# hanzz2007/libxsmm-1

Hardware: AMD Instinct MI355X
Metric: batched SMM fp32 32x32x32 GFLOP/s (whole job) (higher is better)
Workload: dtype f32; 1 GPU; configs[1]: batched dense SMM fp32 M=N=K=32 alpha=1 beta=1, batch=1048576 per GPU, strided addressing, MFMA on; batch_per_gpu=1048576, parallelism=batch-shard x1

## Files before the change

include/libxsmm_amd.h:

```cpp
#ifndef LIBXSMM_AMD_H
#define LIBXSMM_AMD_H

#if !defined(LIBXSMM_H)
# include "libxsmm.h"
#endif

LIBXSMM_API int libxsmm_amd_device_count(void);
LIBXSMM_API void libxsmm_amd_set_stream(void* hip_stream);
LIBXSMM_API void* libxsmm_amd_get_stream(void);
LIBXSMM_API void libxsmm_amd_defer_begin(void);
LIBXSMM_API void libxsmm_amd_defer_end(void);
LIBXSMM_API int libxsmm_amd_defer_active(void);
LIBXSMM_API void libxsmm_amd_flush(void);
LIBXSMM_API int libxsmm_amd_merge_segments(int n, const unsigned long long hulls[], int segment_of[]);
LIBXSMM_API int libxsmm_amd_merge_last_plan(int* ncalls, int* nsegments, int* ndevice_hulls, unsigned long long hulls[], int segment_of[], int capacity);
LIBXSMM_API int libxsmm_amd_smm_plan_describe(const libxsmm_gemm_descriptor* descriptor, int mode, int sync, long long batch,
  long long stride_a, long long stride_b, long long stride_c, unsigned int address_bits, int relaxed, long long uniform_run, int mfma, int lowp,
  char* buffer, size_t buffer_size, int compile_tiles);
LIBXSMM_API int libxsmm_amd_synchronize(void);
LIBXSMM_API void* libxsmm_amd_device_malloc(size_t size);
LIBXSMM_API void libxsmm_amd_device_free(void* ptr);
LIBXSMM_API int libxsmm_amd_memcpy_h2d(void* dst_device, const void* src_host, size_t size);
LIBXSMM_API int libxsmm_amd_memcpy_d2h(void* dst_host, const void* src_device, size_t size);
LIBXSMM_API int libxsmm_amd_is_device_pointer(const void* ptr);

LIBXSMM_API int libxsmm_amd_set_mfma(int mode);
LIBXSMM_API int libxsmm_amd_get_mfma(void);
LIBXSMM_API const char* libxsmm_amd_last_kernel(void);
LIBXSMM_API unsigned long long libxsmm_amd_launch_count(void);
LIBXSMM_API unsigned long long libxsmm_amd_jit_launch_count(void);

LIBXSMM_API int libxsmm_amd_stream_probe(const void* a, const void* b, void* c, long long bytes);

LIBXSMM_API int libxsmm_amd_gemm_batch_strided(const libxsmm_gemm_descriptor* descriptor,
  const void* a, const void* b, void* c, long long stride_a, long long stride_b, long long stride_c,
  long long batchsize);

LIBXSMM_API int libxsmm_amd_gemm_batch_groups(libxsmm_gemm_precision iprec, libxsmm_gemm_precision oprec, int ngroups,
  const char transa[], const char transb[], const libxsmm_blasint m[], const libxsmm_blasint n[], const libxsmm_blasint k[],
  const libxsmm_blasint lda[], const libxsmm_blasint ldb[], const libxsmm_blasint ldc[], const void* alpha, const void* beta,
  const void* const a[], const void* const b[], void* const c[], libxsmm_blasint index_base, libxsmm_blasint index_stride,
  const libxsmm_blasint* const stride_a[], const libxsmm_blasint* const stride_b[], const libxsmm_blasint* const stride_c[],
  const libxsmm_blasint group_size[], int relaxed);

typedef struct libxsmm_amd_spmdm_batch libxsmm_amd_spmdm_batch;
LIBXSMM_API libxsmm_amd_spmdm_batch* libxsmm_amd_spmdm_batch_create(int M, int N, int K, long long batch);
LIBXSMM_API void libxsmm_amd_spmdm_batch_destroy(libxsmm_amd_spmdm_batch* sb);
LIBXSMM_API int libxsmm_amd_spmdm_batch_create_slices(libxsmm_amd_spmdm_batch* sb, char transa, const float* a);
LIBXSMM_API int libxsmm_amd_spmdm_batch_compute(libxsmm_amd_spmdm_batch* sb, char transb, const float* b,
  char transc, const float* beta, float* c);
LIBXSMM_API int libxsmm_amd_spmdm_batch_get_slice(const libxsmm_amd_spmdm_batch* sb, long long item,
  uint16_t* rowidx, uint16_t* colidx, float* values, int capacity);

LIBXSMM_API int libxsmm_amd_spmdm_createSparseSlice_all(const libxsmm_spmdm_handle* handle, char transa, const float* a,
  libxsmm_CSR_sparseslice* libxsmm_output_csr_a);
LIBXSMM_API int libxsmm_amd_spmdm_compute_all(const libxsmm_spmdm_handle* handle, char transa, char transb, const float* alpha,
  libxsmm_CSR_sparseslice* a_sparse, const float* b, char transc, const float* beta, float* c);
LIBXSMM_API int libxsmm_amd_spmdm_createSparseSlice_bfloat16_all(const libxsmm_spmdm_handle* handle, char transa, const libxsmm_bfloat16* a,
  libxsmm_CSR_sparseslice* libxsmm_output_csr_a);
LIBXSMM_API int libxsmm_amd_spmdm_compute_bfloat16_all(const libxsmm_spmdm_handle* handle, char transa, char transb, const libxsmm_bfloat16* alpha,
  libxsmm_CSR_sparseslice* a_sparse, const libxsmm_bfloat16* b, char transc, const libxsmm_bfloat16* beta, float* c);

LIBXSMM_API int libxsmm_amd_dfsspmdm_execute_batch(const libxsmm_dfsspmdm* handle, const double* B, double* C, long long batch);
LIBXSMM_API int libxsmm_amd_sfsspmdm_execute_batch(const libxsmm_sfsspmdm* handle, const float* B, float* C, long long batch);

LIBXSMM_API int libxsmm_amd_csr_kernel_source(int typesize, int M, int K, const unsigned int* row_ptr, const unsigned int* column_idx,
  const double* values, int beta0, int vec, char* buffer, size_t buffer_size, int compile);

LIBXSMM_API int libxsmm_amd_smm_kernel_source(const libxsmm_gemm_descriptor* descriptor, int variant, char* buffer, size_t buffer_size, int compile);

LIBXSMM_API int libxsmm_amd_smm_grouped_kernel_source(const libxsmm_gemm_descriptor* const descriptors[], int ndescriptors, char* buffer, size_t buffer_size, int compile);

LIBXSMM_API void libxsmm_amd_jit_wait(void);
LIBXSMM_API void libxsmm_amd_jit_drain(void);
LIBXSMM_API int libxsmm_amd_jit_prebuild(const libxsmm_gemm_descriptor* const descriptors[], int ndescriptors, int grouped);

typedef struct libxsmm_amd_spgemm libxsmm_amd_spgemm;
LIBXSMM_API libxsmm_amd_spgemm* libxsmm_amd_spgemm_create(const libxsmm_gemm_descriptor* descriptor, int is_csr,
  const unsigned int* row_idx, const unsigned int* column_idx, int fma);
LIBXSMM_API int libxsmm_amd_spgemm_execute_batch(const libxsmm_amd_spgemm* handle, const void* sparse_values, const void* dense, void* c,
  long long stride_dense, long long stride_c, long long batch);
LIBXSMM_API void libxsmm_amd_spgemm_destroy(const libxsmm_amd_spgemm* handle);
LIBXSMM_API int libxsmm_amd_spgemm_source(const libxsmm_gemm_descriptor* descriptor, int is_csr, const unsigned int* row_idx,
  const unsigned int* column_idx, int fma, char* buffer, size_t buffer_size, int compile);
LIBXSMM_API int libxsmm_amd_soa_source(const libxsmm_gemm_descriptor* descriptor, int form, const unsigned int* ptr, const unsigned int* idx,
  int fma, char* buffer, size_t buffer_size, int compile);

LIBXSMM_API int libxsmm_amd_sparse_reader(const char* path, int is_csr, unsigned int** o_ptr, unsigned int** o_idx, double** o_values,
  unsigned int* o_row_count, unsigned int* o_column_count, unsigned int* o_element_count);

LIBXSMM_API int libxsmm_amd_soa_width(libxsmm_gemm_precision precision);
LIBXSMM_API int libxsmm_amd_kernel_execute_batch(const void* kernel, const void* a, const void* b, void* c,
  long long stride_dense, long long stride_c, long long batch);

LIBXSMM_API int libxsmm_amd_packed_width(unsigned int typesize);
LIBXSMM_API int libxsmm_amd_packed_execute_batch(const void* kernel, const void* a, const void* b, void* c, long long npacks);
LIBXSMM_API int libxsmm_amd_packed_kernel_source(const void* descriptor, int kind, char* buffer, size_t buffer_size, int compile);

LIBXSMM_API int libxsmm_amd_matcopy_batch(void* out, const void* in, unsigned int typesize, libxsmm_blasint m, libxsmm_blasint n,
  libxsmm_blasint ldi, libxsmm_blasint ldo, long long stride_in, long long stride_out, long long batch);
LIBXSMM_API int libxsmm_amd_otrans_batch(void* out, const void* in, unsigned int typesize, libxsmm_blasint m, libxsmm_blasint n,
  libxsmm_blasint ldi, libxsmm_blasint ldo, long long stride_in, long long stride_out, long long batch);
LIBXSMM_API int libxsmm_amd_matcopy_batch_ptr(void* const out[], const void* const in[], unsigned int typesize, libxsmm_blasint m,
  libxsmm_blasint n, libxsmm_blasint ldi, libxsmm_blasint ldo, long long batch);
LIBXSMM_API int libxsmm_amd_otrans_batch_ptr(void* const out[], const void* const in[], unsigned int typesize, libxsmm_blasint m,
  libxsmm_blasint n, libxsmm_blasint ldi, libxsmm_blasint ldo, long long batch);

LIBXSMM_API int libxsmm_amd_gemm_task(const libxsmm_gemm_handle* handle, int tid, int nthreads, unsigned int rect[4]);
LIBXSMM_API int libxsmm_amd_gemm_tile(void);

LIBXSMM_API int libxsmm_amd_lowp_gemm(libxsmm_gemm_precision iprec, libxsmm_gemm_precision oprec, char transa, char transb,
  libxsmm_blasint m, libxsmm_blasint n, libxsmm_blasint k, const void* a, libxsmm_blasint lda, const void* b, libxsmm_blasint ldb,
  int beta, void* c, libxsmm_blasint ldc);
LIBXSMM_API int libxsmm_amd_lowp_gemm_thread(libxsmm_gemm_precision iprec, libxsmm_gemm_precision oprec, char transa, char transb,
  libxsmm_blasint m, libxsmm_blasint n, libxsmm_blasint k, const void* a, libxsmm_blasint lda, const void* b, libxsmm_blasint ldb,
  int beta, void* c, libxsmm_blasint ldc, int tid, int nthreads);
LIBXSMM_API int libxsmm_amd_set_lowp_fast(int on);
LIBXSMM_API int libxsmm_amd_get_lowp_fast(void);
LIBXSMM_API int libxsmm_amd_lowp_gemm_chunk(libxsmm_gemm_precision iprec);

LIBXSMM_API int libxsmm_amd_dnn_quantize_async(float* in_buffer, short* out_buffer, int length, unsigned char add_shift, unsigned char* scf, int round_mode);
LIBXSMM_API int libxsmm_amd_dnn_quantize_act_async(float* in_buffer, short* out_buffer, unsigned int N, unsigned int C, unsigned int H, unsigned int W,
  unsigned int cblk_f32, unsigned int cblk_i16, unsigned int lp_blk, unsigned char add_shift, unsigned char* scf, int round_mode);
LIBXSMM_API int libxsmm_amd_dnn_quantize_fil_async(float* in_buffer, short* out_buffer, unsigned int K, unsigned int C, unsigned int R, unsigned int S,
  unsigned int cblk_f32, unsigned int cblk_i16, unsigned int kblk_f32, unsigned int kblk_i16, unsigned int lp_blk, unsigned char add_shift,
  unsigned char* scf, int round_mode);
LIBXSMM_API void libxsmm_amd_dnn_quantize_set_seed(unsigned int seed);

LIBXSMM_API int libxsmm_amd_matdiff_async(libxsmm_matdiff_info* info, libxsmm_datatype datatype, libxsmm_blasint m, libxsmm_blasint n,
  const void* ref, const void* tst, const libxsmm_blasint* ldref, const libxsmm_blasint* ldtst);
LIBXSMM_API int libxsmm_amd_matdiff_batch(libxsmm_matdiff_info* info, libxsmm_matdiff_info* items, long long* item, libxsmm_datatype datatype,
  libxsmm_blasint m, libxsmm_blasint n, const void* ref, const void* tst, const libxsmm_blasint* ldref, const libxsmm_blasint* ldtst,
  long long stride_ref, long long stride_tst, long long batch);

#endif
```

libxsmm-1_amd/csrc/kernels/smm_special.hip:

```cpp
#include "smm_common.cuh"
#include <mutex>

namespace xsmm {
namespace {

typedef float f32x4 __attribute__((ext_vector_type(4)));
typedef float f32x16 __attribute__((ext_vector_type(16)));
typedef double f64x4 __attribute__((ext_vector_type(4)));

__device__ __forceinline__ bool aligned16(const void* p) { return 0 == (reinterpret_cast<uintptr_t>(p) & 15); }

template<bool GLB> struct Space { typedef float* ptr; typedef const float* cptr; typedef f32x4* vptr; typedef const f32x4* cvptr; };
template<> struct Space<true> {
  typedef __attribute__((address_space(1))) float* ptr; typedef const __attribute__((address_space(1))) float* cptr;
  typedef __attribute__((address_space(1))) f32x4* vptr; typedef const __attribute__((address_space(1))) f32x4* cvptr;
};
template<bool NT, bool GLB> __device__ __forceinline__ f32x4 ld4(const float* p, bool al)
{
  const typename Space<GLB>::cptr g = (typename Space<GLB>::cptr)p;
  if (al) return NT ? __builtin_nontemporal_load((typename Space<GLB>::cvptr)g) : *(typename Space<GLB>::cvptr)g;
  return f32x4{ g[0], g[1], g[2], g[3] };
}
template<bool NT, bool GLB> __device__ __forceinline__ void st4(float* p, bool al, f32x4 v)
{
  const typename Space<GLB>::ptr g = (typename Space<GLB>::ptr)p;
  if (al) { if (NT) __builtin_nontemporal_store(v, (typename Space<GLB>::vptr)g); else *(typename Space<GLB>::vptr)g = v; }
  else { g[0] = v[0]; g[1] = v[1]; g[2] = v[2]; g[3] = v[3]; }
}
template<bool NT, bool GLB> __device__ __forceinline__ float ld1(const float* p) { const typename Space<GLB>::cptr g = (typename Space<GLB>::cptr)p; return NT ? __builtin_nontemporal_load(g) : *g; }
template<bool NT, bool GLB> __device__ __forceinline__ void st1(float* p, float v) { const typename Space<GLB>::ptr g = (typename Space<GLB>::ptr)p; if (NT) __builtin_nontemporal_store(v, g); else *g = v; }

template<bool NT, bool GLB> __device__ __forceinline__ void load_mat32(const float* p, int lane, f32x4 (&r)[4])
{
  const bool al = aligned16(p);
#pragma unroll
  for (int j = 0; j < 4; ++j) r[j] = ld4<NT, GLB>(p + 4 * (64 * j + lane), al);
}

template<int KEYSHIFT> __device__ __forceinline__ void park_ab(float* As, float* Bs, int lane, const f32x4 (&ra)[4], const f32x4 (&rb)[4])
{
#pragma unroll
  for (int j = 0; j < 4; ++j) {
    const int c = 64 * j + lane;
    *reinterpret_cast<f32x4*>(As + 4 * c) = ra[j];
    const int n = c >> 3, q = c & 7;
    *reinterpret_cast<f32x4*>(Bs + 4 * (n * 8 + (q ^ ((n >> KEYSHIFT) & 7)))) = rb[j];
  }
}

template<bool BETA0, bool NT, bool GLB>
__global__ __launch_bounds__(256, 4)
void smm32_f32_fma_kernel(DevAddr ad, long long batch)
{
  __shared__ __align__(16) float lds[4][2048];
  const int wave = __builtin_amdgcn_readfirstlane(threadIdx.x >> 6), lane = threadIdx.x & 63;
  const int tx = lane & 7, ty = lane >> 3;
  float* const As = lds[wave];
  float* const Bs = lds[wave] + 1024;
  const long long w = (long long)blockIdx.x * 4 + wave, W = (long long)gridDim.x * 4;
  if (w >= batch) return;

  f32x4 ra[4], rb[4], rc[4];
  load_mat32<NT, GLB>(addr_a<float>(ad, w), lane, ra);
  load_mat32<NT, GLB>(addr_b<float>(ad, w), lane, rb);
  if (!BETA0) {
    const float* const pc = addr_c<float>(ad, w) + 4 * ty * 32 + 4 * tx;
    const bool al = aligned16(pc);
#pragma unroll
    for (int j = 0; j < 4; ++j) rc[j] = ld4<NT, GLB>(pc + j * 32, al);
  }
  for (long long item = w; item < batch; item += W) {
    float* const pc = addr_c<float>(ad, item) + 4 * ty * 32 + 4 * tx;
    park_ab<2>(As, Bs, lane, ra, rb);
    f32x4 acc[4];
#pragma unroll
    for (int j = 0; j < 4; ++j) acc[j] = BETA0 ? f32x4{ 0.f, 0.f, 0.f, 0.f } : rc[j];
    const long long next = item + W;
    if (next < batch) {
      load_mat32<NT, GLB>(addr_a<float>(ad, next), lane, ra);
      load_mat32<NT, GLB>(addr_b<float>(ad, next), lane, rb);
      if (!BETA0) {
        const float* const pn = addr_c<float>(ad, next) + 4 * ty * 32 + 4 * tx;
        const bool al = aligned16(pn);
#pragma unroll
        for (int j = 0; j < 4; ++j) rc[j] = ld4<NT, GLB>(pn + j * 32, al);
      }
    }
    wave_lds_sync();
#pragma unroll 2
    for (int q = 0; q < 8; ++q) {
      f32x4 av[4], bv[4];
#pragma unroll
      for (int kk = 0; kk < 4; ++kk) av[kk] = *reinterpret_cast<const f32x4*>(As + (4 * q + kk) * 32 + 4 * tx);
#pragma unroll
      for (int j = 0; j < 4; ++j) bv[j] = *reinterpret_cast<const f32x4*>(Bs + 4 * ((4 * ty + j) * 8 + (q ^ ty)));
#pragma unroll
      for (int kk = 0; kk < 4; ++kk) {
#pragma unroll
        for (int j = 0; j < 4; ++j) {
#pragma unroll
          for (int i = 0; i < 4; ++i) acc[j][i] = xfma(av[kk][i], bv[j][kk], acc[j][i]);
        }
      }
    }
    const bool al = aligned16(pc);
#pragma unroll
    for (int j = 0; j < 4; ++j) st4<NT, GLB>(pc + j * 32, al, acc[j]);
    wave_lds_sync();
  }
}

template<bool BETA0, bool NT, bool GLB, bool RUNS>
__global__ __launch_bounds__(256, 4)
void smm32_f32_mfma_kernel(DevAddr ad, long long batch, int runlen)
{
  __shared__ __align__(16) float lds[4][2048];
  const int wave = __builtin_amdgcn_readfirstlane(threadIdx.x >> 6), lane = threadIdx.x & 63;
  const int lo = lane & 31, hi = lane >> 5;
  float* const As = lds[wave];
  float* const Bs = lds[wave] + 1024;
  const long long w = (long long)blockIdx.x * 4 + wave, W = (long long)gridDim.x * 4;
  const long long nunits = RUNS ? batch / runlen : batch;
  if (w >= nunits) return;
  const int coff = 4 * hi * 32 + lo;

  f32x4 ra[4], rb[4];
  float rc[16];
  auto load_c = [&](const float* pc) {
#pragma unroll
    for (int r = 0; r < 16; ++r) rc[r] = ld1<NT, GLB>(pc + ((r & 3) + 8 * (r >> 2)) * 32);
  };
  long long unit = w;
  int r0 = 0;
  auto step = [&](long long u, int r, long long& u1, int& r1) { r1 = RUNS ? r + 1 : 0; u1 = u; if (!RUNS || r1 == runlen) { r1 = 0; u1 += W; } };
  float* pc_cur; float* pc_nxt = nullptr;
  {
    const long long first = RUNS ? unit * runlen : unit;
    load_mat32<NT, GLB>(addr_a<float>(ad, first), lane, ra);
    load_mat32<NT, GLB>(addr_b<float>(ad, first), lane, rb);
    pc_cur = addr_c<float>(ad, first);
    if (!BETA0) load_c(pc_cur + coff);
  }
  long long raw_a = 0, raw_b = 0, raw_c = 0;
  if (!RUNS && unit + W < nunits) {
    raw_a = raw_of(ad.a, ad.ia, ad.sa, ad, unit + W); raw_b = raw_of(ad.b, ad.ib, ad.sb, ad, unit + W); raw_c = raw_of(ad.c, ad.ic, ad.sc, ad, unit + W);
  }
  f32x16 acc;
  f32x16 pend; float* pend_pc = nullptr;
  auto store_pend = [&]() {
#pragma unroll
    for (int r = 0; r < 16; ++r) st1<NT, GLB>(pend_pc + ((r & 3) + 8 * (r >> 2)) * 32, pend[r]);
  };
  for (;;) {
    __builtin_amdgcn_s_waitcnt(0x0F70);
    if (nullptr != pend_pc) { store_pend(); pend_pc = nullptr; }
    park_ab<1>(As, Bs, lane, ra, rb);
    if (!RUNS || 0 == r0) {
#pragma unroll
      for (int r = 0; r < 16; ++r) acc[r] = BETA0 ? 0.f : rc[r];
    }
    int r1; long long unit1; step(unit, r0, unit1, r1);
    const bool more = unit1 < nunits;
    if (more) {
      if (RUNS) {
        const long long next = unit1 * runlen + r1;
        load_mat32<NT, GLB>(addr_a<float>(ad, next), lane, ra);
        load_mat32<NT, GLB>(addr_b<float>(ad, next), lane, rb);
        if (0 == r1) { pc_nxt = addr_c<float>(ad, next); if (!BETA0) load_c(pc_nxt + coff); } else pc_nxt = pc_cur;
      }
      else {
        load_mat32<NT, GLB>(cooked<const float>(ad.a, ad, raw_a), lane, ra);
        load_mat32<NT, GLB>(cooked<const float>(ad.b, ad, raw_b), lane, rb);
        pc_nxt = cooked<float>(ad.c, ad, raw_c);
        if (!BETA0) load_c(pc_nxt + coff);
        const long long next2 = unit1 + W;
        if (next2 < nunits) { raw_a = raw_of(ad.a, ad.ia, ad.sa, ad, next2); raw_b = raw_of(ad.b, ad.ib, ad.sb, ad, next2); raw_c = raw_of(ad.c, ad.ic, ad.sc, ad, next2); }
      }
    }
    wave_lds_sync();
    f32x4 bt[8];
#pragma unroll
    for (int t = 0; t < 8; ++t) bt[t] = *reinterpret_cast<const f32x4*>(Bs + 4 * (lo * 8 + (t ^ ((lo >> 1) & 7))));
#pragma unroll
    for (int s = 0; s < 16; ++s) {
      const float av = As[(2 * s + hi) * 32 + lo];
      const float bv = (0 != hi) ? bt[s >> 1][2 * (s & 1) + 1] : bt[s >> 1][2 * (s & 1)];
      acc = __builtin_amdgcn_mfma_f32_32x32x2f32(bv, av, acc, 0, 0, 0);
    }
    if (!RUNS || r0 + 1 == runlen) { pend = acc; pend_pc = pc_cur + coff; }
    wave_lds_sync();
    if (!more) break;
    unit = unit1; r0 = r1; pc_cur = pc_nxt;
  }
  if (nullptr != pend_pc) store_pend();
}

template<bool BETA0>
__global__ __launch_bounds__(256, 4)
void smm64_f32_mfma_kernel(DevAddr ad, long long batch)
{
  __shared__ __align__(16) float As[4096];
  __shared__ __align__(16) float Bs[4096];
  const int t = threadIdx.x, wave = __builtin_amdgcn_readfirstlane(t >> 6), lane = t & 63, lo = lane & 31, hi = lane >> 5;
  const int mq = wave & 1, nq = wave >> 1;
  const int m = 32 * mq + lo, n = 32 * nq + lo;
  const int coff = (32 * nq + 4 * hi) * 64 + m;
  long long item = blockIdx.x;
  if (item >= batch) return;

  f32x4 ra[4], rb[4];
  float rc[16];
  auto load_ab = [&](long long i) {
    const float* const pa = addr_a<float>(ad, i);
    const float* const pb = addr_b<float>(ad, i);
    const bool ala = aligned16(pa), alb = aligned16(pb);
#pragma unroll
    for (int j = 0; j < 4; ++j) {
      ra[j] = ld4<true, false>(pa + 4 * (256 * j + t), ala);
      rb[j] = ld4<true, false>(pb + 4 * (256 * j + t), alb);
    }
  };
  auto load_c = [&](const float* pc) {
#pragma unroll
    for (int r = 0; r < 16; ++r) rc[r] = ld1<true, false>(pc + ((r & 3) + 8 * (r >> 2)) * 64);
  };
  load_ab(item);
  if (!BETA0) load_c(addr_c<float>(ad, item) + coff);
  for (; item < batch; item += gridDim.x) {
    float* const pc = addr_c<float>(ad, item) + coff;
#pragma unroll
    for (int j = 0; j < 4; ++j) {
      const int c = 256 * j + t, row = c >> 4, q = c & 15;
      *reinterpret_cast<f32x4*>(As + row * 64 + ((4 * q) ^ ((row & 1) << 5))) = ra[j];
      *reinterpret_cast<f32x4*>(Bs + row * 64 + 4 * (q ^ (row & 15))) = rb[j];
    }
    f32x16 acc;
#pragma unroll
    for (int r = 0; r < 16; ++r) acc[r] = BETA0 ? 0.f : rc[r];
    const long long next = item + gridDim.x;
    if (next < batch) {
      load_ab(next);
      if (!BETA0) load_c(addr_c<float>(ad, next) + coff);
    }
    __syncthreads();
#pragma unroll
    for (int half = 0; half < 2; ++half) {
      f32x4 bt[8];
#pragma unroll
      for (int u = 0; u < 8; ++u) bt[u] = *reinterpret_cast<const f32x4*>(Bs + n * 64 + 4 * ((8 * half + u) ^ (n & 15)));
#pragma unroll
      for (int s = 0; s < 16; ++s) {
        const float av = As[(32 * half + 2 * s + hi) * 64 + (m ^ (hi << 5))];
        const float bv = (0 != hi) ? bt[s >> 1][2 * (s & 1) + 1] : bt[s >> 1][2 * (s & 1)];
        acc = __builtin_amdgcn_mfma_f32_32x32x2f32(bv, av, acc, 0, 0, 0);
      }
    }
#pragma unroll
    for (int r = 0; r < 16; ++r) st1<true, false>(pc + ((r & 3) + 8 * (r >> 2)) * 64, acc[r]);
    __syncthreads();
  }
}

#include "smm_mfma_wg.inc"

__global__ __launch_bounds__(256)
void stream_abc_kernel(const f32x4* __restrict__ a, const f32x4* __restrict__ b, f32x4* __restrict__ c, long long items)
{
  const int lane = threadIdx.x & 63;
  const long long w = (long long)blockIdx.x * (blockDim.x >> 6) + __builtin_amdgcn_readfirstlane(threadIdx.x >> 6), W = ((long long)gridDim.x * blockDim.x) >> 6;
  if (w >= items) return;
  f32x4 ra[4], rb[4], rc[4];
#pragma unroll
  for (int j = 0; j < 4; ++j) {
    const long long o = w * 256 + 64 * j + lane;
    ra[j] = __builtin_nontemporal_load(a + o); rb[j] = __builtin_nontemporal_load(b + o); rc[j] = __builtin_nontemporal_load(c + o);
  }
  for (long long it = w; it < items; it += W) {
    f32x4 r[4];
#pragma unroll
    for (int j = 0; j < 4; ++j) r[j] = ra[j] + rb[j] + rc[j];
    const long long nx = it + W;
    if (nx < items) {
#pragma unroll
      for (int j = 0; j < 4; ++j) {
        const long long o = nx * 256 + 64 * j + lane;
        ra[j] = __builtin_nontemporal_load(a + o); rb[j] = __builtin_nontemporal_load(b + o); rc[j] = __builtin_nontemporal_load(c + o);
      }
    }
#pragma unroll
    for (int j = 0; j < 4; ++j) __builtin_nontemporal_store(r[j], c + it * 256 + 64 * j + lane);
  }
}

int env_int(const char* name, int fallback)
{
  const char* const v = getenv(name);
  return (nullptr != v && 0 != *v) ? atoi(v) : fallback;
}

bool is_smm32_f32(const SmmBatch& s)
{
  return 4 == s.typesize && 32 == s.m && 32 == s.n && 32 == s.k && 32 == s.lda && 32 == s.ldb && 32 == s.ldc
      && 0 == (s.flags & LIBXSMM_GEMM_FLAG_TRANS_B) && SYNC_NONE == s.sync && 0 == s.general;
}

bool is_smm64(const SmmBatch& s, int typesize)
{
  return typesize == s.typesize && 64 == s.m && 64 == s.n && 64 == s.k && 64 == s.lda && 64 == s.ldb && 64 == s.ldc
      && 0 == (s.flags & LIBXSMM_GEMM_FLAG_TRANS_B) && SYNC_NONE == s.sync && 0 == s.general && 0 != s.use_mfma;
}

long long mfma_wg_units(const SmmBatch& s)
{
  if (SYNC_NONE == s.sync) return s.batch;
  if (SYNC_RUNS == s.sync && 0 < s.uniform_run && 0 == s.batch % s.uniform_run) return s.batch / s.uniform_run;
  return 0;
}
int mfma_wg_runlen(const SmmBatch& s) { return SYNC_NONE == s.sync ? 1 : s.uniform_run; }

template<bool NT, bool GLB>
int launch_smm32(const SmmBatch& s, hipStream_t st, unsigned blocks, const char** name)
{
  const bool beta0 = (0 != (s.flags & LIBXSMM_GEMM_FLAG_BETA_0));
  const DevAddr ad = make_addr(s);
  if (0 == s.use_mfma) {
    *name = "smm_f32_32x32x32_fma";
    if (beta0) hipLaunchKernelGGL((smm32_f32_fma_kernel<true, NT, GLB>), dim3(blocks), dim3(256), 0, st, ad, s.batch);
    else hipLaunchKernelGGL((smm32_f32_fma_kernel<false, NT, GLB>), dim3(blocks), dim3(256), 0, st, ad, s.batch);
  }
  else {
    *name = "smm_f32_32x32x32_mfma";
    if (beta0) hipLaunchKernelGGL((smm32_f32_mfma_kernel<true, NT, GLB, false>), dim3(blocks), dim3(256), 0, st, ad, s.batch, 1);
    else hipLaunchKernelGGL((smm32_f32_mfma_kernel<false, NT, GLB, false>), dim3(blocks), dim3(256), 0, st, ad, s.batch, 1);
  }
  return (int)hipGetLastError();
}

}

int launch_smm_special(const SmmBatch& s, void* stream, const char** name)
{
  hipStream_t st = (hipStream_t)stream;
  if (is_smm32_f32(s)) {
    const int bpc = env_int("XSMM_SMM32_BPC", (ADDR_STRIDED == s.mode || 0 == s.use_mfma) ? 3 : 4), nt = env_int("XSMM_SMM32_NT", 1);
    const int variant = env_int("XSMM_SMM32_VARIANT", 0 != s.use_mfma ? 0 : 1);
    long long blocks = (s.batch + 3) / 4;
    const int grid_env = env_int("XSMM_SMM32_GRID", 0);
    const long long resident = (0 < grid_env) ? grid_env : 256LL * (bpc > 0 ? bpc : 3);
    if (blocks > resident) blocks = resident;
    if (1 == variant) return (0 != nt) ? launch_smm32<true, true>(s, st, (unsigned)blocks, name) : launch_smm32<false, true>(s, st, (unsigned)blocks, name);
    return (0 != nt) ? launch_smm32<true, false>(s, st, (unsigned)blocks, name) : launch_smm32<false, false>(s, st, (unsigned)blocks, name);
  }
  if (4 == s.typesize && 32 == s.m && 32 == s.n && 32 == s.k && 32 == s.lda && 32 == s.ldb && 32 == s.ldc && 0 == (s.flags & LIBXSMM_GEMM_FLAG_TRANS_B)
    && SYNC_RUNS == s.sync && 0 < s.uniform_run && 0 == s.batch % s.uniform_run && 0 == s.general && 0 != s.use_mfma && 0 != env_int("XSMM_SMM32_RUNS", 1))
  {
    const long long units = s.batch / s.uniform_run;
    const int bpc = env_int("XSMM_SMM32_RUNS_BPC", 4);
    long long blocks = (units + 3) / 4;
    const long long resident = 256LL * (bpc > 0 ? bpc : 4);
    if (blocks > resident) blocks = resident;
    if (blocks < 1) return -1;
    const DevAddr ad = make_addr(s);
    *name = "smm_f32_32x32x32_mfma_runs";
    if (0 != (s.flags & LIBXSMM_GEMM_FLAG_BETA_0)) hipLaunchKernelGGL((smm32_f32_mfma_kernel<true, false, true, true>), dim3((unsigned)blocks), dim3(256), 0, st, ad, s.batch, s.uniform_run);
    else hipLaunchKernelGGL((smm32_f32_mfma_kernel<false, false, true, true>), dim3((unsigned)blocks), dim3(256), 0, st, ad, s.batch, s.uniform_run);
    return (int)hipGetLastError();
  }
  if (is_smm64(s, 4) && 0 != env_int("XSMM_SMM64_MFMA", 1) && 0 != env_int("XSMM_SMM64_TIGHT", 1)) {
    const int bpc = env_int("XSMM_SMM64_BPC", 4);
    long long blocks = s.batch;
    const long long resident = 256LL * (bpc > 0 ? bpc : 3);
    if (blocks > resident) blocks = resident;
    if (blocks < 1) return -1;
    const DevAddr ad = make_addr(s);
    *name = "smm_f32_64x64x64_mfma";
    if (0 != (s.flags & LIBXSMM_GEMM_FLAG_BETA_0)) hipLaunchKernelGGL((smm64_f32_mfma_kernel<true>), dim3((unsigned)blocks), dim3(256), 0, st, ad, s.batch);
    else hipLaunchKernelGGL((smm64_f32_mfma_kernel<false>), dim3((unsigned)blocks), dim3(256), 0, st, ad, s.batch);
    return (int)hipGetLastError();
  }
  if (4 == s.typesize && (32 < s.m || 32 < s.n) && s.m <= 64 && s.n <= 64 && 0 < s.k && s.k <= 64 && s.lda >= s.m && s.ldb >= s.k && s.ldc >= s.m
    && 0 == (s.flags & LIBXSMM_GEMM_FLAG_TRANS_B) && mfma_wg_units(s) > 0 && 0 == s.general && 0 != s.use_mfma && 0 != env_int("XSMM_SMM64_MFMA", 1))
  {
    const bool tightc = s.ldc == s.m && 0 == ((s.m * s.n) & 3) && 0 != (s.m & 31) && 0 != env_int("XSMM_SMM64_TIGHTC", 1);
    const int bpc = env_int("XSMM_SMM64_BPC", tightc ? 3 : 4);
    long long blocks = mfma_wg_units(s);
    const long long resident = 256LL * (bpc > 0 ? bpc : 4);
    if (blocks > resident) blocks = resident;
    if (blocks < 1) return -1;
    const DevAddr ad = make_addr(s);
    const int runlen = mfma_wg_runlen(s);
    *name = (1 == runlen) ? "smm_f32_mfma_wg" : "smm_f32_mfma_wg_runs";
    const bool beta0 = 0 != (s.flags & LIBXSMM_GEMM_FLAG_BETA_0);
    const bool tight = s.lda == s.m && s.ldb == s.k && 0 == ((s.m * s.k) & 3) && 0 == ((s.k * s.n) & 3) && 0 != env_int("XSMM_SMM64_WIDE", 1);
#define XSMM_MW(B0, TI, TC) hipLaunchKernelGGL((smm_f32_mfma_wg_kernel<B0, TI, TC>), dim3((unsigned)blocks), dim3(256), 0, st, ad, s.m, s.n, s.k, s.lda, s.ldb, s.ldc, s.batch, runlen)
    if (tightc) { if (tight) { if (beta0) XSMM_MW(true, true, true); else XSMM_MW(false, true, true); } else { if (beta0) XSMM_MW(true, false, true); else XSMM_MW(false, false, true); } }
    else { if (tight) { if (beta0) XSMM_MW(true, true, false); else XSMM_MW(false, true, false); } else { if (beta0) XSMM_MW(true, false, false); else XSMM_MW(false, false, false); } }
#undef XSMM_MW
    return (int)hipGetLastError();
  }
  if (8 == s.typesize && (32 < s.m || 32 < s.n) && s.m <= 64 && s.n <= 64 && 0 < s.k && s.k <= 64 && s.lda >= s.m && s.ldb >= s.k && s.ldc >= s.m
    && 0 == (s.flags & LIBXSMM_GEMM_FLAG_TRANS_B) && mfma_wg_units(s) > 0 && 0 == s.general && 0 != s.use_mfma && 0 != env_int("XSMM_SMM64_MFMA", 1))
  {
    const bool two = s.k > 32 && 0 != env_int("XSMM_SMM64_TWOSTAGE", 1);
    const size_t lds = two ? (size_t)2 * 32 * 64 * sizeof(double) : (size_t)2 * (4 * ((s.k + 3) / 4)) * 64 * sizeof(double);
    int fit = (int)((160u * 1024u) / lds);
    if (fit > 3) fit = 3;
    const int bpc = env_int("XSMM_SMM64_BPC", fit);
    long long blocks = mfma_wg_units(s);
    const long long resident = 256LL * (bpc > 0 ? bpc : fit);
    if (blocks > resident) blocks = resident;
    if (blocks < 1) return -1;
    const DevAddr ad = make_addr(s);
    const int runlen = mfma_wg_runlen(s);
    *name = (1 == runlen) ? "smm_f64_mfma_wg" : "smm_f64_mfma_wg_runs";
    static std::once_flag once;
    std::call_once(once, []() {
      (void)hipFuncSetAttribute(reinterpret_cast<const void*>(&smm_f64_mfma_wg_kernel<true>), hipFuncAttributeMaxDynamicSharedMemorySize, 64 * 1024);
      (void)hipFuncSetAttribute(reinterpret_cast<const void*>(&smm_f64_mfma_wg_kernel<false>), hipFuncAttributeMaxDynamicSharedMemorySize, 64 * 1024);
    });
    if (two) {
      if (0 != (s.flags & LIBXSMM_GEMM_FLAG_BETA_0)) hipLaunchKernelGGL((smm_f64_mfma_wg2_kernel<true>), dim3((unsigned)blocks), dim3(256), lds, st, ad, s.m, s.n, s.k, s.lda, s.ldb, s.ldc, s.batch, runlen);
      else hipLaunchKernelGGL((smm_f64_mfma_wg2_kernel<false>), dim3((unsigned)blocks), dim3(256), lds, st, ad, s.m, s.n, s.k, s.lda, s.ldb, s.ldc, s.batch, runlen);
      return (int)hipGetLastError();
    }
    if (0 != (s.flags & LIBXSMM_GEMM_FLAG_BETA_0)) hipLaunchKernelGGL((smm_f64_mfma_wg_kernel<true>), dim3((unsigned)blocks), dim3(256), lds, st, ad, s.m, s.n, s.k, s.lda, s.ldb, s.ldc, s.batch, runlen);
    else hipLaunchKernelGGL((smm_f64_mfma_wg_kernel<false>), dim3((unsigned)blocks), dim3(256), lds, st, ad, s.m, s.n, s.k, s.lda, s.ldb, s.ldc, s.batch, runlen);
    return (int)hipGetLastError();
  }
  return -1;
}

int launch_stream_abc(const void* a, const void* b, void* c, long long bytes, void* stream)
{
  const long long items = bytes / 4096;
  const int bpc = env_int("XSMM_STREAM_BPC", 3);
  hipLaunchKernelGGL(stream_abc_kernel, dim3(256u * (unsigned)(bpc > 0 ? bpc : 3)), dim3(256), 0, (hipStream_t)stream,
    (const f32x4*)a, (const f32x4*)b, (f32x4*)c, items);
  return (int)hipGetLastError();
}

}
```

Before: 23310 GFLOP/s.

## Add specialized strided 32x32x32 MFMA kernel with software-pipelined prefetch

Adds a dedicated strided-address kernel for fp32 32x32x32 MFMA batches with aligned pointers. It precomputes byte strides, uses nontemporal vector loads and stores, and prefetches the next item's A/B/C into registers while computing the current one. The C store of each item is deferred into the next iteration. The prefetch depth is a template parameter selectable by env, and with the default depth 0 the loads are issued one unit at a time with explicit waitcnts. The default path activates whenever the inputs are aligned and strided, so the generic kernel is bypassed. This risks register pressure and serialized waits.

```diff
diff --git a/include/libxsmm_amd.h b/include/libxsmm_amd.h
--- a/include/libxsmm_amd.h
+++ b/include/libxsmm_amd.h
@@ -29,6 +29,7 @@
 LIBXSMM_API const char* libxsmm_amd_last_kernel(void);
 LIBXSMM_API unsigned long long libxsmm_amd_launch_count(void);
 LIBXSMM_API unsigned long long libxsmm_amd_jit_launch_count(void);
+LIBXSMM_API int libxsmm_amd_smm32_path(void);
 
 LIBXSMM_API int libxsmm_amd_stream_probe(const void* a, const void* b, void* c, long long bytes);
 
diff --git a/libxsmm-1_amd/csrc/kernels/smm_special.hip b/libxsmm-1_amd/csrc/kernels/smm_special.hip
--- a/libxsmm-1_amd/csrc/kernels/smm_special.hip
+++ b/libxsmm-1_amd/csrc/kernels/smm_special.hip
@@ -195,6 +195,86 @@
   if (nullptr != pend_pc) store_pend();
 }
 
+struct Strided32 { const char* a; const char* b; char* c; long long sa, sb, sc; };
+constexpr int SMM32_FAST_DEPTH = 0, SMM32_FAST_BPC = 3;
+
+template<bool BETA0, int DEPTH>
+__global__ __launch_bounds__(256, 4)
+void smm32_f32_mfma_kernel_strided(Strided32 ad, long long batch)
+{
+  typedef const __attribute__((address_space(1))) char* gcbytes;
+  typedef __attribute__((address_space(1))) char* gbytes;
+  __shared__ __align__(16) float lds[4][2048];
+  const int wave = __builtin_amdgcn_readfirstlane(threadIdx.x >> 6), lane = threadIdx.x & 63;
+  const int lo = lane & 31, hi = lane >> 5;
+  float* const As = lds[wave];
+  float* const Bs = lds[wave] + 1024;
+  const long long w = (long long)blockIdx.x * 4 + wave, W = (long long)gridDim.x * 4;
+  if (w >= batch) return;
+  const unsigned abyte = 16u * (unsigned)lane;
+  const unsigned cbyte = 4u * (unsigned)(4 * hi * 32 + lo);
+  f32x4 ra[4], rb[4];
+  float rc[16];
+  auto request = [&](long long item, int u0, int u1) {
+    const gcbytes pa = (gcbytes)(ad.a + item * ad.sa), pb = (gcbytes)(ad.b + item * ad.sb), pc = (gcbytes)(ad.c + item * ad.sc);
+#pragma unroll
+    for (int u = 0; u < 12; ++u) {
+      if (u < u0 || u >= u1) continue;
+      if (u < 4) ra[u] = __builtin_nontemporal_load((Space<true>::cvptr)(pa + abyte + 1024 * u));
+      else if (u < 8) rb[u - 4] = __builtin_nontemporal_load((Space<true>::cvptr)(pb + abyte + 1024 * (u - 4)));
+      else if (!BETA0) {
+#pragma unroll
+        for (int r = 4 * (u - 8); r < 4 * (u - 8) + 4; ++r) rc[r] = __builtin_nontemporal_load((Space<true>::cptr)(pc + cbyte + 128 * ((r & 3) + 8 * (r >> 2))));
+      }
+    }
+  };
+  f32x16 acc, pend;
+  auto store_pend = [&](long long item) {
+    const gbytes pc = (gbytes)(ad.c + item * ad.sc);
+#pragma unroll
+    for (int r = 0; r < 16; ++r) __builtin_nontemporal_store(pend[r], (Space<true>::ptr)(pc + cbyte + 128 * ((r & 3) + 8 * (r >> 2))));
+  };
+  request(w, 0, 12);
+  long long item = w;
+  for (;;) {
+    __builtin_amdgcn_s_waitcnt(0x0F70);
+    if (item != w) store_pend(item - W);
+    park_ab<1>(As, Bs, lane, ra, rb);
+#pragma unroll
+    for (int r = 0; r < 16; ++r) acc[r] = BETA0 ? 0.f : rc[r];
+    const long long next = item + W;
+    const bool more = next < batch;
+    if (more) {
+      if (0 == DEPTH) {
+#pragma unroll
+        for (int u = 0; u < 8; ++u) { __builtin_amdgcn_s_waitcnt(0x0F70); request(next, u, u + 1); }
+        request(next, 8, 12);
+        __builtin_amdgcn_s_waitcnt(0x0F70);
+      }
+      else request(next, 0, DEPTH);
+    }
+    wave_lds_sync();
+    f32x4 bt[8];
+#pragma unroll
+    for (int t = 0; t < 8; ++t) bt[t] = *reinterpret_cast<const f32x4*>(Bs + 4 * (lo * 8 + (t ^ ((lo >> 1) & 7))));
+#pragma unroll
+    for (int s = 0; s < 16; ++s) {
+      const float av = As[(2 * s + hi) * 32 + lo];
+      const float bv = (0 != hi) ? bt[s >> 1][2 * (s & 1) + 1] : bt[s >> 1][2 * (s & 1)];
+      acc = __builtin_amdgcn_mfma_f32_32x32x2f32(bv, av, acc, 0, 0, 0);
+    }
+    pend = acc;
+    wave_lds_sync();
+    if (!more) break;
+    if (0 < DEPTH && DEPTH < 12) {
+      __builtin_amdgcn_sched_barrier(0);
+      request(next, DEPTH, 12);
+    }
+    item = next;
+  }
+  store_pend(item);
+}
+
 template<bool BETA0>
 __global__ __launch_bounds__(256, 4)
 void smm64_f32_mfma_kernel(DevAddr ad, long long batch)
@@ -336,12 +416,52 @@
   return (int)hipGetLastError();
 }
 
+thread_local int tl_smm32_path = -1;
+
+bool smm32_strided_aligned(const SmmBatch& s)
+{
+  return ADDR_STRIDED == s.mode
+      && 0 == ((reinterpret_cast<uintptr_t>(s.a) | reinterpret_cast<uintptr_t>(s.b) | reinterpret_cast<uintptr_t>(s.c)
+              | (uintptr_t)(4 * s.sa) | (uintptr_t)(4 * s.sb) | (uintptr_t)(4 * s.sc)) & 15);
+}
+
+template<int DEPTH>
+int launch_smm32_strided(const SmmBatch& s, hipStream_t st, unsigned blocks)
+{
+  const Strided32 ad = { (const char*)s.a, (const char*)s.b, (char*)s.c, 4 * s.sa, 4 * s.sb, 4 * s.sc };
+  if (0 != (s.flags & LIBXSMM_GEMM_FLAG_BETA_0)) hipLaunchKernelGGL((smm32_f32_mfma_kernel_strided<true, DEPTH>), dim3(blocks), dim3(256), 0, st, ad, s.batch);
+  else hipLaunchKernelGGL((smm32_f32_mfma_kernel_strided<false, DEPTH>), dim3(blocks), dim3(256), 0, st, ad, s.batch);
+  return (int)hipGetLastError();
+}
+
 }
 
 int launch_smm_special(const SmmBatch& s, void* stream, const char** name)
 {
   hipStream_t st = (hipStream_t)stream;
   if (is_smm32_f32(s)) {
+    tl_smm32_path = -1;
+    if (0 != s.use_mfma && smm32_strided_aligned(s) && 0 != env_int("XSMM_SMM32_FAST", 1) && 0 != env_int("XSMM_SMM32_NT", 1)
+      && nullptr == getenv("XSMM_SMM32_VARIANT"))
+    {
+      const int bpc = env_int("XSMM_SMM32_BPC", SMM32_FAST_BPC), grid_env = env_int("XSMM_SMM32_GRID", 0);
+      const int depth = env_int("XSMM_SMM32_DEPTH", SMM32_FAST_DEPTH);
+      long long blocks = (s.batch + 3) / 4;
+      const long long resident = (0 < grid_env) ? grid_env : 256LL * (bpc > 0 ? bpc : SMM32_FAST_BPC);
+      if (blocks > resident) blocks = resident;
+      *name = "smm_f32_32x32x32_mfma";
+      int e;
+      switch (depth) {
+        case 0: e = launch_smm32_strided<0>(s, st, (unsigned)blocks); break;
+        case 2: e = launch_smm32_strided<2>(s, st, (unsigned)blocks); break;
+        case 4: e = launch_smm32_strided<4>(s, st, (unsigned)blocks); break;
+        case 8: e = launch_smm32_strided<8>(s, st, (unsigned)blocks); break;
+        case 12: e = launch_smm32_strided<12>(s, st, (unsigned)blocks); break;
+        default: return (int)hipErrorInvalidValue;
+      }
+      tl_smm32_path = depth;
+      return e;
+    }
     const int bpc = env_int("XSMM_SMM32_BPC", (ADDR_STRIDED == s.mode || 0 == s.use_mfma) ? 3 : 4), nt = env_int("XSMM_SMM32_NT", 1);
     const int variant = env_int("XSMM_SMM32_VARIANT", 0 != s.use_mfma ? 0 : 1);
     long long blocks = (s.batch + 3) / 4;
@@ -440,3 +560,5 @@
 }
 
 }
+
+LIBXSMM_API int libxsmm_amd_smm32_path(void) { return xsmm::tl_smm32_path; }
```

After: 23230 GFLOP/s. About the same (-0.3%).
